# distributed-lab/linea-stark-prover

Hardware: AMD Instinct MI355X
Metric: prove time (s) + trace-rows/sec, 3x3 perm AIR @2^19; NTT HBM GB/s vs roofline (higher is better)
Workload: dtype fr253 (BLS12-377 Fr, 8x u32 Montgomery limbs); 1 GPU; 3x3 permutation AIR, 2^19 rows (w=8, q=4 quotient chunks, log_blowup 3, 33 queries, Poseidon2-w3 Merkle, FRI); log_n=19, width=8, fri_queries=33, parallelism=single-gpu

## Files before the change

linea_stark_prover_amd/csrc/capi.cpp:

```cpp
#include <hip/hip_runtime.h>

#include <algorithm>
#include <cstdlib>
#include <cstring>
#include <memory>
#include <thread>

#include "comm.hpp"
#include "prove_internal.hpp"

using namespace lsp;

namespace {
thread_local std::string g_err;

#ifdef LSP_DEBUG_BOUNDS
std::string bounds_fault_report() {
    int n = 0;
    if (hipGetDeviceCount(&n) != hipSuccess || n == 0) return "";
    (void)hipDeviceSynchronize();
    static const char* const files[] = {"k_ntt.hip", "k_hash.hip", "k_field.hip", "k_quotient.hip", "k_open.hip",
                                        "k_witness.hip", "k_check.hip", "fr29.hpp", "k_common.hpp", "poseidon2_f29.hpp",
                                        "fr.hpp"};
    static unsigned (*const readers[])() = {bounds_fault_k_ntt, bounds_fault_k_hash, bounds_fault_k_field,
// ... 92 lines not shown
                uint64_t x = next();
                c.v[2 * k] = (uint32_t)x;
                c.v[2 * k + 1] = (uint32_t)(x >> 32);
            }
            c.v[7] &= (1u << 29) - 1;
            if (fr_words_lt_mod(c)) return fr_from_canonical(c);
        }
    }
    uint64_t below(uint64_t n) {
        const unsigned __int128 two64 = (unsigned __int128)1 << 64;
        const unsigned __int128 lim = two64 - (two64 % n);
        for (;;) {
            uint64_t x = next();
            if ((unsigned __int128)x < lim) return x % n;
        }
    }
};
}

extern "C" {

#ifdef LSP_DEBUG_BOUNDS
const char* lsp_version(void) { return "linea_stark_prover_amd 0.1 (gfx950, debug-bounds)"; }
#else
const char* lsp_version(void) { return "linea_stark_prover_amd 0.1 (gfx950)"; }
#endif

int lsp_debug_bounds_probe(lsp_ctx* ctx) {
    return guarded(ctx, [&] {
        LSP_REQUIRE(ctx, LSP_E_ARG, "null ctx");
        std::lock_guard<std::mutex> g(ctx->mu);
        need_gpu(ctx);
#ifndef LSP_DEBUG_BOUNDS
        throw LspError(LSP_E_STATE, "not a debug-bounds build (python -m linea_stark_prover_amd.build --debug-bounds)");
#else
        uint32_t* sink = (uint32_t*)ctx->buf("bounds_probe", 4 * sizeof(uint32_t));
        LSP_HIP(launch_bounds_probe(sink, ctx->stream));
        ctx->sync();
#endif
    });
}

int lsp_device_count(int* n) {
    return guarded(nullptr, [&] {
        LSP_REQUIRE(n, LSP_E_ARG, "null");
        int c = 0;
        if (hipGetDeviceCount(&c) != hipSuccess) c = 0;
        *n = c;
    });
}

const char* lsp_last_error(const lsp_ctx* ctx) { return ctx ? ctx->err.c_str() : g_err.c_str(); }

int lsp_seeded_setup(uint64_t seed, uint32_t rounds_f, uint32_t rounds_p, lsp_fr* alpha, lsp_fr* delta,
                     lsp_fr* rc) {
    return guarded(nullptr, [&] {
        LSP_REQUIRE(alpha && delta && rc && rounds_f % 2 == 0, LSP_E_ARG, "bad seeded_setup arguments");
        SplitMix64 g{seed};
        *alpha = from_fr(g.fr());
        *delta = from_fr(g.fr());
        for (uint32_t i = 0; i < 3 * rounds_f + rounds_p; ++i) rc[i] = from_fr(g.fr());
    });
}

void lsp_fr_from_canonical(const uint64_t in[4], lsp_fr* out) {
    if (!in || !out) return;
    lsp_fr t;
    std::memcpy(t.l, in, 32);
    *out = from_fr(fr_from_canonical(to_fr(t)));
}
void lsp_fr_to_canonical(const lsp_fr* in, uint64_t out[4]) {
    if (!in || !out) return;
    lsp_fr t = from_fr(fr_to_canonical(to_fr(*in)));
    std::memcpy(out, t.l, 32);
}
void lsp_fr_from_be_bytes_mod_order(const uint8_t* be, size_t n, lsp_fr* out) {
    if (!out || (!be && n)) return;
    const Fr b256 = fr_from_u64(256);
    Fr acc = fr_zero();
    for (size_t i = 0; i < n; ++i) acc = fr_add(fr_mul(acc, b256), fr_from_u64(be[i]));
    *out = from_fr(acc);
}
void lsp_fr_mul(const lsp_fr* a, const lsp_fr* b, lsp_fr* out) {
    if (a && b && out) *out = from_fr(fr_mul(to_fr(*a), to_fr(*b))); }
void lsp_fr_inv(const lsp_fr* a, lsp_fr* out) {
    if (a && out) *out = from_fr(fr_inv(to_fr(*a)));
}
void lsp_two_adic_generator(uint32_t bits, lsp_fr* out) {
    if (!out) return;
    if (bits > 47) bits = 47;
    *out = from_fr(host_two_adic_generator(bits));
}

int lsp_ctx_create(int device, const lsp_params* p, lsp_ctx** out) {
    return guarded(nullptr, [&] {
        LSP_REQUIRE(p && out && p->round_constants, LSP_E_ARG, "null params");
        LSP_REQUIRE(p->struct_size == sizeof(lsp_params), LSP_E_ARG,
                    "lsp_params.struct_size must be sizeof(lsp_params) of this header (caller built against "
                    "another lsp.h?)");
        LSP_REQUIRE(p->skip_log_degree <= 1 && p->skip_public_values <= 1 && p->observe_opened_values <= 1 &&
                        p->sample_bits_montgomery <= 1 && p->skip_final_poly <= 1,
                    LSP_E_ARG, "transcript switches are 0 or 1");
        LSP_REQUIRE(p->sbox_degree == 11 || p->sbox_degree == 17, LSP_E_ARG, "S-box degree must be 11 or 17");
        LSP_REQUIRE(p->rounds_f >= 2 && p->rounds_f % 2 == 0 && p->rounds_f <= 64 && p->rounds_p <= 256, LSP_E_ARG,
                    "bad round counts");
        LSP_REQUIRE(p->log_blowup >= 1 && p->log_blowup <= 8 && p->num_queries >= 1 && p->num_queries <= 1024 &&
                        p->proof_of_work_bits <= 32 && p->log_final_poly_len <= 8 &&
                        (p->public_degree == 0 || p->public_degree == 1),
                    LSP_E_ARG, "bad FRI parameters");
        auto c = std::make_unique<lsp_ctx>();
        c->device = device;
        c->p2.L = P2Layout{p->rounds_f, p->rounds_p, p->sbox_degree};
        const size_t nround = 3 * p->rounds_f + p->rounds_p;
        const size_t nrc = nround + P2_LIN_N;
        c->p2.rc.resize(nrc);
        for (size_t i = 0; i < nround; ++i) c->p2.rc[i] = to_fr(p->round_constants[i]);
        {
            static const uint32_t dm[9] = {2, 1, 1, 1, 2, 1, 1, 1, 2}, dd[3] = {1, 1, 2};
            bool gen = false;
            for (int k = 0; k < 9; ++k) {
                const Fr def = fr_from_u64(dm[k]);
                Fr v = def;
                if (p->external_mds) {
                    v = to_fr(p->external_mds[k]);
                    LSP_REQUIRE(fr_words_lt_mod(v), LSP_E_ARG, "external_mds entry not canonical");
                }
                gen |= !fr_eq(v, def);
                c->p2.rc[nround + k] = v;
            }
            for (int k = 0; k < 3; ++k) {
                const Fr def = fr_from_u64(dd[k]);
                Fr v = def;
                if (p->internal_diag) {
                    v = to_fr(p->internal_diag[k]);
                    LSP_REQUIRE(fr_words_lt_mod(v), LSP_E_ARG, "internal_diag entry not canonical");
                }
                gen |= !fr_eq(v, def);
                c->p2.rc[nround + 9 + k] = v;
            }
            c->p2.L.gen_lin = gen ? 1u : 0u;
        }
        if (ifma::available()) ifma::prepare(c->p2.rc, c->p2.rc8);
        if (device != LSP_HOST_ONLY) {
            int n = 0;
            if (hipGetDeviceCount(&n) != hipSuccess || n == 0) throw LspError(LSP_E_STATE, "no HIP device");
            LSP_REQUIRE(device >= 0 && device < n, LSP_E_ARG, "bad device index");
            LSP_HIP(hipSetDevice(device));
            LSP_HIP(hipStreamCreateWithFlags(&c->stream, hipStreamNonBlocking));
            int lds = 0;
            if (hipDeviceGetAttribute(&lds, hipDeviceAttributeMaxSharedMemoryPerBlock, device) == hipSuccess && lds > 0)
                c->lds_per_block = (size_t)lds;
            LSP_HIP(hipMalloc(&c->rc_dev, nrc * sizeof(Fr)));
            LSP_HIP(hipMemcpy(c->rc_dev, c->p2.rc.data(), nrc * sizeof(Fr), hipMemcpyHostToDevice));
            LSP_HIP(hipMalloc(&c->rc29_dev, nrc * sizeof(F29)));
            LSP_HIP(launch_rc_to_f29(c->rc_dev, c->rc29_dev, (uint32_t)nrc, c->stream));
            LSP_HIP(hipStreamSynchronize(c->stream));
        }
        c->log_blowup = p->log_blowup;
        c->log_final_poly_len = p->log_final_poly_len;
        c->num_queries = p->num_queries;
        c->pow_bits = p->proof_of_work_bits;
        c->public_degree = p->public_degree;
        c->transcript.log_degree = !p->skip_log_degree;
        c->transcript.public_values = !p->skip_public_values;
        c->transcript.opened_values = p->observe_opened_values != 0;
        c->transcript.mont_bits = p->sample_bits_montgomery != 0;
        c->transcript.final_poly = !p->skip_final_poly;
        *out = c.release();
    });
}

int lsp_ctx_destroy(lsp_ctx* ctx) {
    if (!ctx) return LSP_OK;
    delete ctx->comm;
    ctx->comm = nullptr;
    if (ctx->device == LSP_HOST_ONLY) {
        delete ctx;
        return LSP_OK;
    }
    (void)hipSetDevice(ctx->device);
    (void)hipStreamSynchronize(ctx->stream);
    if (ctx->side_stream) (void)hipStreamSynchronize(ctx->side_stream);
    for (auto& kv : ctx->pool)
        if (kv.second.p) (void)hipFree(kv.second.p);
    for (auto& kv : ctx->hpool)
        if (kv.second.p) (void)hipHostFree(kv.second.p);
    for (auto& kv : ctx->twiddles) (void)hipFree(kv.second);
    for (auto& kv : ctx->stage_ev) (void)hipEventDestroy(kv.second);
    for (hipEvent_t e : ctx->event_pool) (void)hipEventDestroy(e);
    for (auto& t : ctx->pending_timings) {
        (void)hipEventDestroy(std::get<1>(t));
        (void)hipEventDestroy(std::get<2>(t));
    }
    if (ctx->ev_near) (void)hipEventDestroy(ctx->ev_near);
    if (ctx->ev_top) (void)hipEventDestroy(ctx->ev_top);
    if (ctx->ev_warm) (void)hipEventDestroy(ctx->ev_warm);
    if (ctx->side_stream) {
        (void)hipStreamSynchronize(ctx->side_stream);
        (void)hipEventDestroy(ctx->ev_wide);
        (void)hipEventDestroy(ctx->ev_side);
        (void)hipStreamDestroy(ctx->side_stream);
    }
    if (ctx->rc_dev) (void)hipFree(ctx->rc_dev);
    if (ctx->rc29_dev) (void)hipFree(ctx->rc29_dev);
    (void)hipStreamDestroy(ctx->stream);
    delete ctx;
    return LSP_OK;
}

int lsp_synchronize(lsp_ctx* ctx) {
    return guarded(ctx, [&] {
        LSP_REQUIRE(ctx, LSP_E_ARG, "null ctx");
        need_gpu(ctx);
        LSP_HIP(hipDeviceSynchronize());
    });
}

int lsp_dev_alloc(lsp_ctx* ctx, size_t bytes, void** dptr) {
    return guarded(ctx, [&] {
        LSP_REQUIRE(ctx && dptr, LSP_E_ARG, "null");
        need_gpu(ctx);
        if (hipMalloc(dptr, bytes ? bytes : 1) != hipSuccess) {
            (void)hipGetLastError();
            throw LspError(LSP_E_OOM, "hipMalloc failed");
        }
    });
}
int lsp_dev_free(lsp_ctx* ctx, void* dptr) {
    return guarded(ctx, [&] {
        need_gpu(ctx);
        LSP_HIP(hipFree(dptr));
    });
}
int lsp_memcpy_h2d(lsp_ctx* ctx, void* dst, const void* src, size_t bytes) {
    return guarded(ctx, [&] {
        LSP_REQUIRE(ctx && ((dst && src) || bytes == 0), LSP_E_ARG, "null memcpy argument");
        std::lock_guard<std::mutex> g(ctx->mu);
        need_gpu(ctx);
        LSP_HIP(hipMemcpyAsync(dst, src, bytes, hipMemcpyHostToDevice, ctx->stream));
        ctx->sync();
    });
}
int lsp_memcpy_d2h(lsp_ctx* ctx, void* dst, const void* src, size_t bytes) {
    return guarded(ctx, [&] {
        LSP_REQUIRE(ctx && ((dst && src) || bytes == 0), LSP_E_ARG, "null memcpy argument");
        std::lock_guard<std::mutex> g(ctx->mu);
        need_gpu(ctx);
        LSP_HIP(hipMemcpyAsync(dst, src, bytes, hipMemcpyDeviceToHost, ctx->stream));
        ctx->sync();
    });
}

int lsp_coset_lde_batch_shifts(lsp_ctx* ctx, const lsp_fr* in, size_t h, size_t w, uint32_t added_bits,
                               const lsp_fr* shifts, lsp_fr* out, int mem) {
    return guarded(ctx, [&] {
        LSP_REQUIRE(ctx && shifts && w >= 1, LSP_E_ARG, "bad arguments");
        std::lock_guard<std::mutex> g(ctx->mu);
        need_gpu(ctx);
        log2_exact(h);
        LSP_REQUIRE(added_bits <= 16, LSP_E_ARG, "added_bits too large");
        const size_t N = h << added_bits;
        std::vector<Fr> sh(w);
        for (size_t c = 0; c < w; ++c) sh[c] = to_fr(shifts[c]);
        const Fr* din = dev_in(ctx, in, h * w, mem, "api_in");
        Fr* dout = dev_out(ctx, out, N * w, mem, "api_out");
        lde_device(ctx, din, h, w, added_bits, sh.data(), dout);
        finish_out(ctx, out, dout, N * w, mem);
    });
}

int lsp_coset_lde_batch(lsp_ctx* ctx, const lsp_fr* in, size_t h, size_t w, uint32_t added_bits,
                        const lsp_fr* shift, lsp_fr* out, int mem) {
    if (!shift || w == 0) return LSP_E_ARG;
    std::vector<lsp_fr> sh(w, *shift);
    return lsp_coset_lde_batch_shifts(ctx, in, h, w, added_bits, sh.data(), out, mem);
}

int lsp_coset_dft_batch(lsp_ctx* ctx, const lsp_fr* coeffs, size_t h, size_t w, const lsp_fr* shift, lsp_fr* out,
                        int mem) {
    return guarded(ctx, [&] {
        LSP_REQUIRE(ctx && w >= 1, LSP_E_ARG, "bad dft arguments");
        std::lock_guard<std::mutex> g(ctx->mu);
        need_gpu(ctx);
        log2_exact(h);
        const Fr s = shift ? to_fr(*shift) : fr_one();
        const Fr* din = dev_in(ctx, coeffs, h * w, mem, "api_in");
        Fr* dout = dev_out(ctx, out, h * w, mem, "api_out");
        coset_dft_device(ctx, din, h, w, s, dout);
        finish_out(ctx, out, dout, h * w, mem);
    });
}

int lsp_coset_idft_batch(lsp_ctx* ctx, const lsp_fr* evals, size_t h, size_t w, const lsp_fr* shift, lsp_fr* out,
                         int mem) {
    return guarded(ctx, [&] {
        LSP_REQUIRE(ctx && w >= 1, LSP_E_ARG, "bad idft arguments");
        std::lock_guard<std::mutex> g(ctx->mu);
        need_gpu(ctx);
        log2_exact(h);
        const Fr s = shift ? to_fr(*shift) : fr_one();
        LSP_REQUIRE(!fr_is_zero(fr_to_canonical(s)), LSP_E_ARG, "coset shift must be nonzero");
        const Fr* din = dev_in(ctx, evals, h * w, mem, "api_in");
        Fr* dout = dev_out(ctx, out, h * w, mem, "api_out");
        coset_idft_device(ctx, din, h, w, s, dout);
        finish_out(ctx, out, dout, h * w, mem);
    });
}
// ... 1139 lines not shown
```

linea_stark_prover_amd/csrc/k_hash.hip:

```cpp
#include <cstdlib>

#include "k_common.hpp"
#include "kernels.hpp"
#include "poseidon2_f29.hpp"
#include "poseidon2_row.hpp"

namespace lsp {

#ifndef LSP_P2_ROWS_WPE
#define LSP_P2_ROWS_WPE 1
#endif

namespace {
template <uint32_t D>
__global__ __launch_bounds__(256) void k_permute(Fr* __restrict__ st, size_t n, const F29* __restrict__ rc,
                                                 uint32_t rf, uint32_t rp) {
    __shared__ uint4 qt[3 * F29_QTAB_N];
    f29_qtab_init(qt);
    __syncthreads();
    const size_t i = gtid();
    if (i >= n) return;
    F29 s0 = f29_from_fr(st[3 * i]), s1 = f29_from_fr(st[3 * i + 1]), s2 = f29_from_fr(st[3 * i + 2]);
    permute3_any<D, 1>(s0, s1, s2, rc, rf, rp, qt);
    st[3 * i] = f29_to_fr(s0);
    st[3 * i + 1] = f29_to_fr(s1);
    st[3 * i + 2] = f29_to_fr(s2);
}

template <uint32_t D, int LANES>
__global__ __launch_bounds__(256) __attribute__((amdgpu_waves_per_eu(LSP_P2_ROWS_WPE))) void k_hash_rows1(const Fr* __restrict__ m, uint32_t w, size_t nrows,
                                                    Fr* __restrict__ out, const F29* __restrict__ rc, uint32_t rf,
                                                    uint32_t rp) {
    __shared__ uint4 qt[3 * F29_QTAB_N];
    f29_qtab_init(qt);
    __syncthreads();
    const size_t i = gtid() / LANES;
    if (i >= nrows) return;
    const Fr* row = m + i * w;
    const Fr d = sponge_f29<D, LANES>([&](uint32_t k) { return LSP_BOUNDS(k < w) ? row[k] : fr_zero(); }, w, rc, rf,
                                      rp, qt);
    if ((threadIdx.x & (LANES - 1)) == 0) out[i] = d;
}

template <uint32_t D, int LANES>
__global__ __launch_bounds__(256) __attribute__((amdgpu_waves_per_eu(LSP_P2_ROWS_WPE))) void k_hash_rows_multi(MatList ml, size_t nrows, Fr* __restrict__ out,
                                                         const F29* __restrict__ rc, uint32_t rf, uint32_t rp) {
    __shared__ uint4 qt[3 * F29_QTAB_N];
    f29_qtab_init(qt);
    __syncthreads();
    const size_t i = gtid() / LANES;
    if (i >= nrows) return;
    uint32_t total = 0;
    for (uint32_t j = 0; j < ml.n; ++j) total += ml.width[j];
    auto get = [&](uint32_t k) {
        uint32_t j = 0;
        while (k >= ml.width[j]) {
            k -= ml.width[j];
            ++j;
            if (!LSP_BOUNDS(j < ml.n)) return fr_zero();
        }
        return ml.ptr[j][i * ml.width[j] + k];
    };
    const Fr d = sponge_f29<D, LANES>(get, total, rc, rf, rp, qt);
    if ((threadIdx.x & (LANES - 1)) == 0) out[i] = d;
}

template <uint32_t D, int LANES>
__global__ __launch_bounds__(256) void k_fold_hash(FoldSpec f, size_t nleaves, Fr* __restrict__ out,
                                                   const F29* __restrict__ rc, uint32_t rf, uint32_t rp) {
    __shared__ uint4 qt[3 * F29_QTAB_N];
    f29_qtab_init(qt);
    __syncthreads();
    const size_t j = gtid() / LANES;
    if (j >= nleaves) return;
    Fr e[2];
#pragma unroll
    for (int k = 0; k < 2; ++k) {
        const size_t i = 2 * j + k;
        const Fr p = fr_mul(f.half_beta, pow2l(f.tab, f.L1, brev_bits(f.i0 + i, f.logm)));
        e[k] = fr_add(fr_mul(fr_add(f.half, p), f.v[2 * i]), fr_mul(fr_sub(f.half, p), f.v[2 * i + 1]));
    }
    if ((threadIdx.x & (LANES - 1)) == 0) {
        f.vout[2 * j] = e[0];
        f.vout[2 * j + 1] = e[1];
    }
    const Fr d = sponge_f29<D, LANES>([&](uint32_t k) { return e[k]; }, 2, rc, rf, rp, qt);
    if ((threadIdx.x & (LANES - 1)) == 0) out[j] = d;
}

template <uint32_t D, int LANES>
__global__ __launch_bounds__(256) void k_merkle_level(const Fr* __restrict__ src, Fr* __restrict__ dst, size_t nout,
                                                      const F29* __restrict__ rc, uint32_t rf, uint32_t rp) {
    if constexpr (LANES > 1) __builtin_amdgcn_s_setprio(3);
    __shared__ uint4 qt[3 * F29_QTAB_N];
    f29_qtab_init(qt);
    __syncthreads();
    const size_t i = gtid() / LANES;
    if (i >= nout) return;
    if (!LSP_BOUNDS(2 * i + 1 < 2 * nout)) return;
    const Fr d = compress_f29<D, LANES>(src[2 * i], src[2 * i + 1], rc, rf, rp, qt);
    if ((threadIdx.x & (LANES - 1)) == 0) dst[i] = d;
}

template <uint32_t D>
__global__ __launch_bounds__(64) void k_merkle_level_row(const Fr* __restrict__ src, Fr* __restrict__ dst,
                                                         size_t nout, const F29* __restrict__ rc, uint32_t rf,
                                                         uint32_t rp) {
    __builtin_amdgcn_s_setprio(3);
    __shared__ prow::RowLds tab;
    prow::row_lds_init(&tab);
    __syncthreads();
    const size_t i = blockIdx.x;
    if (i >= nout) return;
    const Fr d = prow::compress_row<D>(src + 2 * i, src + 2 * i + 1, rc, rf, rp, &tab);
    if (threadIdx.x == 0) dst[i] = d;
}

template <uint32_t D>
__global__ __launch_bounds__(256) void k_merkle_top(Fr* __restrict__ layers, size_t off, uint32_t len,
                                                    const F29* __restrict__ rc, uint32_t rf, uint32_t rp) {
    __shared__ uint4 qt[3 * F29_QTAB_N];
    f29_qtab_init(qt);
    __syncthreads();
    __shared__ Fr buf[128];
    if (!LSP_BOUNDS(len <= 128)) return;
    for (uint32_t e = threadIdx.x; e < len; e += blockDim.x) buf[e] = layers[off + e];
    __syncthreads();
    size_t out_off = off + len;
    const uint32_t q = threadIdx.x >> 2;
    const bool lead = (threadIdx.x & 3) == 0;
    while (len > 1) {
        const uint32_t nout = len / 2;
        Fr r;
        if (q < nout) r = compress_f29<D, 4>(buf[2 * q], buf[2 * q + 1], rc, rf, rp, qt);
        __syncthreads();
        if (q < nout && lead) {
            buf[q] = r;
            layers[out_off + q] = r;
        }
        __syncthreads();
        out_off += nout;
        len = nout;
    }
}
template <uint32_t D>
__global__ __launch_bounds__(256) void k_grind(Fr pre0, Fr pre1, Fr pre2, uint32_t wlane, uint64_t base,
                                               uint64_t count, uint32_t bits, uint32_t mont, const F29* __restrict__ rc,
                                               uint32_t rf, uint32_t rp, unsigned long long* __restrict__ best) {
    __shared__ uint4 qt[3 * F29_QTAB_N];
    f29_qtab_init(qt);
    __syncthreads();
    const uint64_t stride = (uint64_t)gridDim.x * blockDim.x;
    const F29 c0 = f29_from_fr(pre0), c1 = f29_from_fr(pre1), c2 = f29_from_fr(pre2);
    const uint64_t mask = bits >= 64 ? ~0ull : ((1ull << bits) - 1);
    for (uint64_t i = gtid(); i < count; i += stride) {
        const uint64_t w = base + i;
        const F29 fw = f29_from_fr(fr_from_u64(w));
        F29 s0 = wlane == 0 ? fw : c0, s1 = wlane == 0 ? c1 : fw, s2 = c2;
        permute3_any<D, 1>(s0, s1, s2, rc, rf, rp, qt);
        const Fr m = f29_to_fr(s0);
        const Fr c = mont ? m : fr_to_canonical(m);
        const uint64_t lo = (uint64_t)c.v[0] | ((uint64_t)c.v[1] << 32);
        if ((lo & mask) == 0) atomicMin(best, (unsigned long long)w);
    }
}

template <uint32_t D>
__global__ __launch_bounds__(256) void k_calib_perm(Fr* __restrict__ out, uint32_t iters, const F29* __restrict__ rc,
                                                    uint32_t rf, uint32_t rp) {
    __shared__ uint4 qt[3 * F29_QTAB_N];
    f29_qtab_init(qt);
    __syncthreads();
    const size_t t = gtid();
    F29 s0 = f29_from_fr(fr_from_u64(t + 1)), s1 = f29_from_fr(fr_from_u64(3 * t + 7)), s2 = f29_zero();
    for (uint32_t i = 0; i < iters; ++i) permute3_any<D, 1>(s0, s1, s2, rc, rf, rp, qt);
    out[t] = f29_to_fr(s0);
}

__global__ void k_rc_to_f29(const Fr* __restrict__ rc, F29* __restrict__ rc29, uint32_t n) {
    const uint32_t i = (uint32_t)gtid();
    if (i < n) rc29[i] = f29_from_fr(rc[i]);
}
}

hipError_t launch_rc_to_f29(const Fr* rc, F29* rc29, uint32_t n, hipStream_t st) {
    hipLaunchKernelGGL(k_rc_to_f29, dim3(nblocks(n, 64)), dim3(64), 0, st, rc, rc29, n);
    return hipGetLastError();
}

#define LSP_DISPATCH_D(L, KERNEL, ...)                                  \
    do {                                                                \
        if ((L).gen_lin) {                                              \
            if ((L).sbox_degree == 17)                                  \
                hipLaunchKernelGGL(KERNEL<17u | P2_GEN>, __VA_ARGS__);  \
            else                                                        \
                hipLaunchKernelGGL(KERNEL<11u | P2_GEN>, __VA_ARGS__);  \
        } else if ((L).sbox_degree == 17)                               \
            hipLaunchKernelGGL(KERNEL<17>, __VA_ARGS__);                \
        else                                                            \
            hipLaunchKernelGGL(KERNEL<11>, __VA_ARGS__);                \
    } while (0)

#define LSP_DISPATCH_DL(DEG, LANES, KERNEL, ...)                          \
    do {                                                                  \
        if ((LANES) == 4)                                                 \
            hipLaunchKernelGGL((KERNEL<DEG, 4>), __VA_ARGS__);            \
        else if ((LANES) == 2)                                            \
            hipLaunchKernelGGL((KERNEL<DEG, 2>), __VA_ARGS__);            \
        else                                                              \
            hipLaunchKernelGGL((KERNEL<DEG, 1>), __VA_ARGS__);            \
    } while (0)
#define LSP_DISPATCH_DC(L, LANES, KERNEL, ...)                            \
    do {                                                                  \
        if ((L).gen_lin) {                                                \
            if ((L).sbox_degree == 17)                                    \
                LSP_DISPATCH_DL(17u | P2_GEN, LANES, KERNEL, __VA_ARGS__);\
            else                                                          \
                LSP_DISPATCH_DL(11u | P2_GEN, LANES, KERNEL, __VA_ARGS__);\
        } else if ((L).sbox_degree == 17)                                 \
            LSP_DISPATCH_DL(17u, LANES, KERNEL, __VA_ARGS__);             \
        else                                                              \
            LSP_DISPATCH_DL(11u, LANES, KERNEL, __VA_ARGS__);             \
    } while (0)

static size_t coop_max() {
    static const size_t v = [] {
        const char* e = std::getenv("LSP_COOP_MAX");
        return e ? (size_t)std::strtoull(e, nullptr, 10) : (size_t)16384;
    }();
    return v;
}
static unsigned coop_bs() {
    static const unsigned v = [] {
        const char* e = std::getenv("LSP_COOP_BS");
        return e ? (unsigned)std::strtoul(e, nullptr, 10) : 0u;
    }();
    return v;
}
#define COOP_MAX coop_max()
static size_t pair_max() {
    static const size_t v = [] {
        const char* e = std::getenv("LSP_PAIR_MAX");
        return e ? (size_t)std::strtoull(e, nullptr, 10) : (size_t)32768;
    }();
    return v;
}
static inline int lanes_for(size_t n) { return n <= COOP_MAX ? 4 : (n <= pair_max() ? 2 : 1); }

static inline void state_grid(size_t n, int lanes, unsigned& blocks, unsigned& bs) {
    if (lanes == 4) {
        bs = coop_bs() ? coop_bs() : (4 * n >= 65536 ? 256u : 64u);
        blocks = nblocks(4 * n, bs);
    } else {
        bs = 256;
        blocks = nblocks((size_t)lanes * n, bs);
    }
}

hipError_t launch_permute(Fr* states, size_t n, const F29* rc, P2Layout L, hipStream_t st) {
    if (!n) return hipSuccess;
    LSP_DISPATCH_D(L, k_permute, dim3(nblocks(n, 256)), dim3(256), 0, st, states, n, rc, L.rounds_f, L.rounds_p);
    return hipGetLastError();
}

hipError_t launch_hash_rows(const MatList& m, size_t nrows, Fr* out, const F29* rc, P2Layout L, hipStream_t st) {
    if (!nrows) return hipSuccess;
    const int lanes = lanes_for(nrows);
    unsigned blocks, bs;
    state_grid(nrows, lanes, blocks, bs);
    if (m.n == 1)
        LSP_DISPATCH_DC(L, lanes, k_hash_rows1, dim3(blocks), dim3(bs), 0, st, m.ptr[0], m.width[0], nrows, out, rc,
                        L.rounds_f, L.rounds_p);
    else
        LSP_DISPATCH_DC(L, lanes, k_hash_rows_multi, dim3(blocks), dim3(bs), 0, st, m, nrows, out, rc, L.rounds_f,
                        L.rounds_p);
    return hipGetLastError();
}

hipError_t launch_fold_hash(const FoldSpec& f, size_t nleaves, Fr* out, const F29* rc, P2Layout L, hipStream_t st) {
    if (!nleaves) return hipSuccess;
    const int lanes = lanes_for(nleaves);
    unsigned blocks, bs;
    state_grid(nleaves, lanes, blocks, bs);
    LSP_DISPATCH_DC(L, lanes, k_fold_hash, dim3(blocks), dim3(bs), 0, st, f, nleaves, out, rc, L.rounds_f, L.rounds_p);
    return hipGetLastError();
}

hipError_t launch_calib_perm(Fr* out, size_t nthreads, uint32_t iters, const F29* rc, P2Layout L, hipStream_t st) {
    LSP_DISPATCH_D(L, k_calib_perm, dim3(nblocks(nthreads, 256)), dim3(256), 0, st, out, iters, rc, L.rounds_f,
                   L.rounds_p);
    return hipGetLastError();
}

hipError_t launch_grind(const Fr pre[3], uint32_t wlane, uint64_t base, uint64_t count, uint32_t bits, bool mont,
                        const F29* rc, P2Layout L, unsigned long long* best, hipStream_t st) {
    const unsigned blocks = 256 * 16;
    LSP_DISPATCH_D(L, k_grind, dim3(blocks), dim3(256), 0, st, pre[0], pre[1], pre[2], wlane, base, count, bits,
                   (uint32_t)mont, rc,
                   L.rounds_f, L.rounds_p, best);
    return hipGetLastError();
}

static size_t row_max() {
    static const size_t v = [] {
        const char* e = std::getenv("LSP_ROW_MAX");
        return e ? (size_t)std::strtoull(e, nullptr, 10) : (size_t)1024;
    }();
    return v;
}

hipError_t launch_merkle_level(const Fr* src, Fr* dst, size_t nout, const F29* rc, P2Layout L, hipStream_t st) {
    if (!nout) return hipSuccess;
    if (!L.gen_lin && nout <= row_max()) {
        if (L.sbox_degree == 17)
            hipLaunchKernelGGL(k_merkle_level_row<17>, dim3((unsigned)nout), dim3(64), 0, st, src, dst, nout, rc,
                               L.rounds_f, L.rounds_p);
        else
            hipLaunchKernelGGL(k_merkle_level_row<11>, dim3((unsigned)nout), dim3(64), 0, st, src, dst, nout, rc,
                               L.rounds_f, L.rounds_p);
        return hipGetLastError();
    }
    const int lanes = lanes_for(nout);
    unsigned blocks, bs;
    state_grid(nout, lanes, blocks, bs);
    LSP_DISPATCH_DC(L, lanes, k_merkle_level, dim3(blocks), dim3(bs), 0, st, src, dst, nout, rc, L.rounds_f,
                    L.rounds_p);
    return hipGetLastError();
}

hipError_t launch_merkle_levels(Fr* layers, size_t nleaves, size_t stop_len, const F29* rc, P2Layout L,
                                size_t* off_out, size_t* len_out, hipStream_t st) {
    size_t off = 0, len = nleaves;
    while (len > stop_len && len > 1) {
        hipError_t e = launch_merkle_level(layers + off, layers + off + len, len / 2, rc, L, st);
        if (e != hipSuccess) return e;
        off += len;
        len /= 2;
    }
    *off_out = off;
    *len_out = len;
    return hipSuccess;
}

hipError_t launch_merkle_tree(Fr* layers, size_t nleaves, const F29* rc, P2Layout L, hipStream_t st) {
    size_t off = 0, len = nleaves;
    while (len > 128) {
        const size_t nout = len / 2;
        hipError_t e = launch_merkle_level(layers + off, layers + off + len, nout, rc, L, st);
        if (e != hipSuccess) return e;
        off += len;
        len /= 2;
    }
    if (len > 1) {
        LSP_DISPATCH_D(L, k_merkle_top, dim3(1), dim3(256), 0, st, layers, off, (uint32_t)len, rc, L.rounds_f,
                       L.rounds_p);
        return hipGetLastError();
    }
    return hipSuccess;
}

}

LSP_BOUNDS_READER(k_hash)
```

linea_stark_prover_amd/csrc/kernels.hpp:

```cpp
#pragma once
#include <hip/hip_runtime.h>
#include <stddef.h>
#include <stdint.h>

#include "fr.hpp"
#include "fr29.hpp"
#include "poseidon2.hpp"

namespace lsp {

constexpr uint32_t COLMAP_PLAIN = 0xffu;
struct ColMap {
    uint32_t logb = COLMAP_PLAIN;
    uint32_t stride = 0, c0 = 0, cstep = 1, valid = 0xffffffffu;
    uint32_t bw = 0;
    static ColMap plain(uint32_t w) {
        ColMap m;
        m.stride = w;
        m.valid = w;
        return m;
    }
    static ColMap blocked(uint32_t logb, uint32_t bw) {
        ColMap m;
        m.logb = logb;
        m.bw = bw;
        return m;
    }
};
hipError_t launch_lde(const Fr* in, Fr* X, Fr* out, size_t w, uint32_t logh, uint32_t ncosets, const uint4* tw_inv,
                      const uint4* tw_fwd, const Fr* twist, uint32_t L1, uint32_t L2, int twist_per_col,
                      const Fr* ratio, hipStream_t st);
hipError_t launch_intt(const Fr* in, ColMap map, Fr* X, size_t w, uint32_t logh, const uint4* tw_inv, hipStream_t st);
hipError_t launch_lde_coeffs(const Fr* coef, ColMap map, Fr* out, size_t w, uint32_t logh, uint32_t ncosets,
                             const uint4* tw_fwd, const Fr* twist, uint32_t L1, uint32_t L2, int twist_per_col,
                             const Fr* ratio, hipStream_t st);
hipError_t launch_fold_subcoset(const Fr* coef, ColMap map, size_t h, size_t S, uint32_t w, const Fr* fac, Fr* out,
                                hipStream_t st);
hipError_t launch_to_f29form(const Fr* in, Fr* out, size_t n, hipStream_t st);
hipError_t launch_scale_coeffs(const Fr* X, size_t h, uint32_t w, const Fr* tab, uint32_t L1, Fr* out,
                               hipStream_t st);
hipError_t launch_to_f29limbs(const Fr* in, uint4* out, size_t n, hipStream_t st);
hipError_t launch_stage_twiddles(const Fr* pw, uint32_t logH, uint4* out, hipStream_t st);
hipError_t launch_pow_tables(const Fr* bases, size_t nbases, uint32_t L1, uint32_t L2, const Fr* scale,
                             Fr* tabs, hipStream_t st);
hipError_t launch_powers(const Fr* tab, uint32_t L1, size_t n, Fr* out, hipStream_t st);

struct MatList {
    const Fr* ptr[8];
    uint32_t width[8];
    uint32_t n;
};
inline MatList one_mat(const Fr* p, uint32_t w) {
    MatList m{};
    m.ptr[0] = p;
    m.width[0] = w;
    m.n = 1;
    return m;
}
hipError_t launch_rc_to_f29(const Fr* rc, F29* rc29, uint32_t n, hipStream_t st);
hipError_t launch_permute(Fr* states, size_t n, const F29* rc29, P2Layout L, hipStream_t st);
struct FoldSpec {
    const Fr* v;
    Fr* vout;
    Fr half, half_beta;
    const Fr* tab;
    uint32_t L1, logm;
    uint64_t i0;
};
hipError_t launch_fold_hash(const FoldSpec& f, size_t nleaves, Fr* out, const F29* rc, P2Layout L, hipStream_t st);
hipError_t launch_hash_rows(const MatList& m, size_t nrows, Fr* out, const F29* rc29, P2Layout L, hipStream_t st);
hipError_t launch_merkle_level(const Fr* src, Fr* dst, size_t nout, const F29* rc29, P2Layout L, hipStream_t st);
hipError_t launch_grind(const Fr pre[3], uint32_t wlane, uint64_t base, uint64_t count, uint32_t bits, bool mont,
                        const F29* rc29, P2Layout L, unsigned long long* best, hipStream_t st);
hipError_t launch_merkle_tree(Fr* layers, size_t nleaves, const F29* rc29, P2Layout L, hipStream_t st);
hipError_t launch_merkle_levels(Fr* layers, size_t nleaves, size_t stop_len, const F29* rc29, P2Layout L,
                                size_t* off_out, size_t* len_out, hipStream_t st);

size_t batch_inverse_scratch(size_t n);
hipError_t launch_batch_inverse(const Fr* in, Fr* out, size_t n, hipStream_t st, Fr* scratch = nullptr,
                                const Fr* inv_total = nullptr);
hipError_t launch_calib_mul(Fr* out, size_t nthreads, uint32_t iters, hipStream_t st);
hipError_t launch_calib_perm(Fr* out, size_t nthreads, uint32_t iters, const F29* rc, P2Layout L, hipStream_t st);
hipError_t launch_gather(const uint64_t* ptrs, Fr* out, size_t n, hipStream_t st);
hipError_t launch_assemble_chunks(const Fr* stage, uint32_t logGq, size_t Sq, Fr* out, hipStream_t st);

size_t witness_scratch_bytes(size_t n, uint32_t ntables);
hipError_t launch_gen_raw_perm(uint64_t seed, size_t n, uint32_t ncols, uint64_t mul, uint64_t add, Fr* a, Fr* b,
                               hipStream_t st);
hipError_t launch_perm_rows(const Fr* a, uint32_t na, const Fr* b, uint32_t nb, size_t n, Fr alpha, Fr delta,
                            Fr* out, size_t ostride, Fr* al, Fr* bl, hipStream_t st);
hipError_t launch_lookup_rows(const Fr* a, uint32_t na, const Fr* b, uint32_t nt, uint32_t nbc, const Fr* afil,
                              const Fr* bfil, size_t n, Fr alpha, Fr delta, Fr* out, size_t ostride, Fr* comb,
                              Fr* den, hipStream_t st);
hipError_t launch_mul_vec(const Fr* x, const Fr* y, size_t n, Fr* out, hipStream_t st);
hipError_t launch_put_col(const Fr* v, size_t n, Fr* out, size_t ostride, uint32_t col, hipStream_t st);
hipError_t launch_fr_scan(const Fr* in, Fr* out, size_t n, bool product, void* scratch, size_t scratch_bytes,
                          hipStream_t st);
hipError_t launch_lookup_occurrences(const Fr* comb, size_t n, uint32_t nt, const Fr* afil, const Fr* bfil,
                                     uint32_t* occ, void* scratch, size_t scratch_bytes, hipStream_t st);
hipError_t launch_lookup_terms(const Fr* inv, const uint32_t* occ, const Fr* afil, size_t n, uint32_t nt, Fr* out,
                               size_t ostride, uint32_t col_ainv, Fr* term, hipStream_t st);

struct QuotientArgs {
    const Fr* lde;
    uint32_t w;
    uint32_t logQ, log_q;
    const int32_t* air;
    uint32_t air_len;
    Fr pub_alpha, pub_delta, alpha;
    Fr gen;
    Fr wh_inv;
    const Fr* tabQ;
    uint32_t L1;
    const Fr* zh;
    const Fr* inv_zh;
    const Fr* inv_den;
    Fr* out;
    uint64_t i0 = 0;
    uint32_t log_step = 0;
    uint64_t row0 = 0;
    uint64_t n = 0;
    const Fr* lde_next = nullptr;
    uint64_t row0_next = 0;
    uint32_t row_order = 0;
    uint64_t lde_rows = 0, lde_next_rows = 0;
    uint32_t* cons = nullptr;
    uint32_t ncons = 0;
    const Fr* pub = nullptr;
    uint32_t npub = 0;
    uint32_t prog = 0, prog_slots = 0;
    const Fr* prep = nullptr;
    uint32_t wp = 0;
};
hipError_t launch_selector_denoms(const Fr* tabQ, uint32_t L1, Fr gen, Fr wh_inv, size_t n, Fr* den,
                                  hipStream_t st, uint64_t i0 = 0, uint32_t log_step = 0);
hipError_t launch_quotient(const QuotientArgs& a, hipStream_t st);
hipError_t launch_quotient_fold(const QuotientArgs& a, hipStream_t st);

struct CheckArgs {
    const Fr* trace;
    uint64_t h;
    uint32_t w;
    const int32_t* air;
    uint32_t ncons;
    Fr pub_alpha, pub_delta;
    uint64_t* row_mask;
    uint64_t* count;
    uint64_t* first_row;
    const uint64_t* rows = nullptr;
    uint32_t nrows = 0;
    Fr* vals = nullptr;
    const Fr* pub = nullptr;
    uint32_t npub = 0;
    uint32_t prog = 0, prog_slots = 0;
    const Fr* prep = nullptr;
    uint32_t wp = 0;
};
hipError_t launch_check(const CheckArgs& a, hipStream_t st);
hipError_t launch_check_rows(const CheckArgs& a, hipStream_t st);

hipError_t launch_open_denoms(Fr z, Fr gen, const Fr* tabN, uint32_t L1, uint32_t logN, size_t n, Fr* den,
                              hipStream_t st, uint64_t row0 = 0);
hipError_t launch_shift_inverse(const Fr* inv_z, Fr* out, Fr c, uint32_t logN, uint64_t step, uint64_t row0, size_t n,
                                hipStream_t st);
hipError_t launch_interp_partial(const Fr* M, uint32_t w, size_t h, const Fr* inv_den, Fr gen, const Fr* tabN,
                                 uint32_t L1, uint32_t logN, Fr* partial, uint32_t* nblocks, hipStream_t st,
                                 uint64_t row0 = 0);
hipError_t launch_sum_partials(const Fr* partial, uint32_t nblocks, uint32_t w, Fr* out, hipStream_t st);
struct ReduceArgs {
    const Fr* lde;
    uint32_t w;
    const Fr* qlde;
    uint32_t q;
    const Fr* inv_z;
    const Fr* inv_zn;
    const Fr* apw;
    Fr ry_z, ry_zn;
    const Fr* ryq;
    Fr* out;
    size_t n;
    F29* consts29 = nullptr;
    size_t lds_max = 64 * 1024;
};
inline size_t reduce_rows_scratch(uint32_t w, uint32_t q, size_t lds_max) {
    const size_t lds = 3 * 64 * 16 + (w + 1 + 2 * (size_t)q) * 36;
    return lds <= lds_max ? 0 : w + 1 + 2 * (size_t)q;
}
hipError_t launch_reduce_rows(const ReduceArgs& a, hipStream_t st);
struct PrepReduceArgs {
    const Fr* prep;
    uint32_t wp;
    const Fr* inv_z;
    const Fr* inv_zn;
    const Fr* apw;
    Fr ry_z, ry_zn, off_z, off_zn;
    Fr* out;
    size_t n;
    size_t lds_max = 64 * 1024;
};
bool reduce_prep_fits(uint32_t wp, size_t lds_max);
hipError_t launch_reduce_prep(const PrepReduceArgs& a, hipStream_t st);
hipError_t launch_bounds_probe(uint32_t* sink, hipStream_t st);
#ifdef LSP_DEBUG_BOUNDS
unsigned bounds_fault_k_ntt();
unsigned bounds_fault_k_hash();
unsigned bounds_fault_k_field();
unsigned bounds_fault_k_quotient();
unsigned bounds_fault_k_open();
unsigned bounds_fault_k_witness();
unsigned bounds_fault_k_check();
#endif
// ... 7 lines not shown
```

linea_stark_prover_amd/csrc/poseidon2_row.hpp:

```cpp
#pragma once
#include "poseidon2_f29.hpp"

namespace lsp {
#include "fr29_row_gfx950.inc"

namespace prow {

__device__ __forceinline__ uint32_t shr1(uint32_t x) {
    return (uint32_t)__builtin_amdgcn_mov_dpp((int)x, 0x111, 0xf, 0xf, true);
}
__device__ __forceinline__ uint32_t bcast8(uint32_t x) {
    return (uint32_t)__builtin_amdgcn_mov_dpp((int)x, 0x158, 0xf, 0xf, false);
}
__device__ __forceinline__ void swap16(uint32_t& a, uint32_t& b) {
    const auto r = __builtin_amdgcn_permlane16_swap(a, b, false, false);
    a = r[0];
    b = r[1];
}
__device__ __forceinline__ void swap32(uint32_t& a, uint32_t& b) {
    const auto r = __builtin_amdgcn_permlane32_swap(a, b, false, false);
    a = r[0];
    b = r[1];
}
__device__ __forceinline__ uint32_t rowsum(uint32_t x) {
    uint32_t a = x, b = x;
    swap16(a, b);
    uint32_t s = a + b, t = s;
    swap32(s, t);
    return s + t;
}
__device__ __forceinline__ uint32_t row0_all(uint32_t x) {
    uint32_t a = x, b = x;
    swap16(a, b);
    uint32_t c = a;
    swap32(a, c);
    return a;
}
__device__ __forceinline__ uint32_t row1_all(uint32_t x) {
    uint32_t a = x, b = x;
    swap16(a, b);
    uint32_t c = b;
    swap32(b, c);
    return b;
}
__device__ __forceinline__ uint32_t row2_all(uint32_t x) {
    uint32_t a = x, b = x;
    swap32(a, b);
    uint32_t c = b;
    swap16(b, c);
    return b;
}

struct Lane {
    F29RowK K;
    uint32_t l;
    uint32_t row;
    bool hi9;
};

__device__ __forceinline__ uint32_t rnorm(uint32_t v, const Lane& L) {
#pragma unroll
    for (int k = 0; k < 2; ++k) v = (v & L.K.maskl) + shr1(v >> 29);
    return L.hi9 ? 0u : v;
}

struct RowLds {
    uint32_t rqt[16 * F29_QTAB_N];
    uint32_t ptab[32];
    uint32_t c0[16];
    uint32_t cto[16];
};

__device__ __forceinline__ void row_lds_init(RowLds* t) {
    for (uint32_t q = threadIdx.x; q < F29_QTAB_N; q += blockDim.x) {
        uint32_t Q[9];
        uint64_t c = 0;
#pragma unroll
        for (int i = 0; i < 8; ++i) {
            const uint64_t v = (uint64_t)q * p29(i) + c;
            Q[i] = (uint32_t)v & F29_MASK;
            c = v >> 29;
        }
        Q[8] = (uint32_t)((uint64_t)q * p29(8) + c);
        uint32_t* e = t->rqt + 16 * q;
        const uint32_t b = q ? 2u : 0u;
        e[0] = q ? (1u << 30) - Q[0] : 0u;
#pragma unroll
        for (int i = 1; i < 8; ++i) e[i] = q ? (1u << 30) - b - Q[i] : 0u;
        e[8] = 0u - b - Q[8];
#pragma unroll
        for (int i = 9; i < 16; ++i) e[i] = 0u;
    }
    constexpr uint32_t TO[9] = {0x1ffffff3u, 0x8e3ffffu, 0x1ffffc9fu, 0xfea1edfu, 0xfee725u,
                                0xabaa896u,  0xa745b60u, 0x6457773u,  0xd4bdau};
    for (uint32_t i = threadIdx.x; i < 32; i += blockDim.x) {
        uint32_t v = 0;
#pragma unroll
        for (int d = 1; d <= 8; ++d) v = i == 8u + d ? p29(d) : v;
        t->ptab[i] = v;
        if (i < 16) {
            uint32_t c = 0, o = 0;
#pragma unroll
            for (int l = 0; l < 9; ++l) {
                c = i == (uint32_t)l ? c29(l) : c;
                o = i == (uint32_t)l ? TO[l] : o;
            }
            t->c0[i] = c;
            t->cto[i] = o;
        }
    }
}

__device__ __forceinline__ Lane row_lane(const RowLds* t) {
    Lane L;
    const uint32_t lane = threadIdx.x & 63u;
    L.l = lane & 15u;
    L.row = lane >> 4;
    L.hi9 = L.l >= 9;
    L.K.c0 = t->c0[L.l];
#pragma unroll
    for (int k = 0; k < 9; ++k) L.K.P[k] = t->ptab[8 + L.l - k];
    L.K.maskl = L.l == 8 ? 0xffffffffu : F29_MASK;
    return L;
}

__device__ __forceinline__ uint32_t rq_entry(uint32_t v, const uint32_t* __restrict__ rqt, const Lane& L) {
    uint32_t q = __umulhi(bcast8(v), 0xdb651d12u) >> 20;
    if (!LSP_BOUNDS(q < F29_QTAB_N)) q = 0;
    q = q ? q - 1 : 0u;
    return rqt[16 * q + L.l];
}
__device__ __forceinline__ uint32_t rreduce(uint32_t v, const uint32_t* __restrict__ rqt, const Lane& L) {
    return rnorm(v + rq_entry(v, rqt, L), L);
}

__device__ __forceinline__ uint32_t rmul(uint32_t a, uint32_t b, const Lane& L) { return f29row_mul(a, b, L.K); }

template <uint32_t D>
__device__ __forceinline__ uint32_t sbox(uint32_t x, const Lane& L) {
    const uint32_t x2 = rmul(x, x, L);
    const uint32_t x4 = rmul(x2, x2, L);
    const uint32_t x8 = rmul(x4, x4, L);
    if (D == 11) return rmul(rmul(x8, x2, L), x, L);
    return rmul(rmul(x8, x8, L), x, L);
}

__device__ __forceinline__ uint32_t load_limb(const Fr* p, const Lane& L) {
    if (L.hi9) return 0u;
    const uint32_t* w = reinterpret_cast<const uint32_t*>(p);
    const uint32_t b = 29 * L.l + 27, W = b >> 5;
    const uint32_t lo = W ? w[W - 1] : 0u, hi = W < 8 ? w[W] : 0u;
    const uint32_t v = __builtin_amdgcn_alignbit(hi, lo, b & 31);
    return L.l < 8 ? v & F29_MASK : v;
}

__device__ __forceinline__ uint32_t rc_limb(const F29* __restrict__ rc29, uint32_t k, const Lane& L) {
    return L.hi9 ? 0u : rc29[k].l[L.l];
}

template <uint32_t D>
__device__ __forceinline__ Fr compress_row(const Fr* left, const Fr* right, const F29* __restrict__ rc29, uint32_t rf,
                                           uint32_t rp, const RowLds* __restrict__ tab) {
    const Lane L = row_lane(tab);
    const uint32_t* rqt = tab->rqt;
    const uint32_t half = rf / 2;
    const F29* ini = rc29;
    const F29* ter = rc29 + 3 * half;
    const F29* itl = rc29 + 6 * half;
    uint32_t S = L.row == 0 ? load_limb(left, L) : L.row == 1 ? load_limb(right, L) : 0u;
    S = rreduce(S, rqt, L);
    uint32_t T = rowsum(S);
    const bool live = L.row < 3;
    uint32_t C = live ? rc_limb(ini, L.row, L) : 0u;
    for (uint32_t r = 0; r < half; ++r) {
        const uint32_t x = rnorm(S + C + T, L);
        C = live && r + 1 < half ? rc_limb(ini, 3 * (r + 1) + L.row, L) : 0u;
        const uint32_t y = sbox<D>(x, L);
        S = live ? y : 0u;
        T = rowsum(S);
    }
    const uint32_t W = S + T;
    uint32_t Ci = rp ? rc_limb(itl, 0, L) : 0u;
    uint32_t X = row0_all(rnorm(W + Ci, L));
    const uint32_t R = rreduce(W, rqt, L);
    uint32_t S1 = row1_all(R), S2 = row2_all(R);
    const bool odd = L.row & 1u;
    uint32_t v1 = S1, v2 = S2, e1 = 0, e2 = 0;
    for (uint32_t r = 0; r < rp; ++r) {
        Ci = r + 1 < rp ? rc_limb(itl, r + 1, L) : 0u;
        const uint32_t x2 = rmul(X, X, L);
        S1 = rnorm(v1 + e1, L);
        S2 = rnorm(v2 + e2, L);
        uint32_t y;
        if (D == 11) {
            uint32_t a = rmul(x2, odd ? X : x2, L);
            uint32_t b = a;
            swap16(a, b);
            y = rmul(rmul(a, a, L), b, L);
        } else {
            const uint32_t x4 = rmul(x2, x2, L);
            const uint32_t x8 = rmul(x4, x4, L);
            y = rmul(rmul(x8, x8, L), X, L);
        }
        const uint32_t u = y + S1 + S2;
        v1 = S1 + u;
        v2 = S2 + S2 + u;
        e1 = rq_entry(v1, rqt, L);
        e2 = rq_entry(v2, rqt, L);
        X = rnorm(y + Ci + u, L);
    }
    S1 = rnorm(v1 + e1, L);
    S2 = rnorm(v2 + e2, L);
    S = L.row == 0 ? X : L.row == 1 ? S1 : L.row == 2 ? S2 : 0u;
    T = 0;
    C = live ? rc_limb(ter, L.row, L) : 0u;
    for (uint32_t r = 0; r < half; ++r) {
        const uint32_t x = rnorm(S + C + T, L);
        C = live && r + 1 < half ? rc_limb(ter, 3 * (r + 1) + L.row, L) : 0u;
        const uint32_t y = sbox<D>(x, L);
        S = live ? y : 0u;
        T = rowsum(S);
    }
    const uint32_t y = rmul(rnorm(S + T, L), tab->cto[L.l], L);
    F29 o;
#pragma unroll
    for (int i = 0; i < 9; ++i) o.l[i] = __builtin_amdgcn_readlane(y, i);
    return fr_reduce_once(f29_repack_out(f29_reduce(o)));
}

}
}
```

Measured before the change: 8.675 million trace-rows/s.

## Precompute row-hash LDS table once and prefetch fold/merkle inputs before table init

```diff
diff --git a/linea_stark_prover_amd/csrc/capi.cpp b/linea_stark_prover_amd/csrc/capi.cpp
--- a/linea_stark_prover_amd/csrc/capi.cpp
+++ b/linea_stark_prover_amd/csrc/capi.cpp
@@ -268,7 +268,7 @@
                 c->lds_per_block = (size_t)lds;
             LSP_HIP(hipMalloc(&c->rc_dev, nrc * sizeof(Fr)));
             LSP_HIP(hipMemcpy(c->rc_dev, c->p2.rc.data(), nrc * sizeof(Fr), hipMemcpyHostToDevice));
-            LSP_HIP(hipMalloc(&c->rc29_dev, nrc * sizeof(F29)));
+            LSP_HIP(hipMalloc(&c->rc29_dev, rc29_bytes(nrc)));
             LSP_HIP(launch_rc_to_f29(c->rc_dev, c->rc29_dev, (uint32_t)nrc, c->stream));
             LSP_HIP(hipStreamSynchronize(c->stream));
         }
diff --git a/linea_stark_prover_amd/csrc/k_hash.hip b/linea_stark_prover_amd/csrc/k_hash.hip
--- a/linea_stark_prover_amd/csrc/k_hash.hip
+++ b/linea_stark_prover_amd/csrc/k_hash.hip
@@ -69,16 +69,44 @@
 __global__ __launch_bounds__(256) void k_fold_hash(FoldSpec f, size_t nleaves, Fr* __restrict__ out,
                                                    const F29* __restrict__ rc, uint32_t rf, uint32_t rp) {
     __shared__ uint4 qt[3 * F29_QTAB_N];
-    f29_qtab_init(qt);
-    __syncthreads();
+    Fr e[2];
+    if constexpr (LANES > 1) {
+        const size_t j = gtid() / LANES;
+        const bool live = j < nleaves;
+        const size_t jl = live ? j : 0;
+        Fr v[4], tl[2], th[2];
+#pragma unroll
+        for (int k = 0; k < 2; ++k) {
+            const size_t i = 2 * jl + k;
+            const uint64_t x = brev_bits(f.i0 + i, f.logm);
+            uint64_t hi = x >> f.L1;
+            if (!LSP_BOUNDS(hi < (1ull << f.L1))) hi = 0;
+            tl[k] = f.tab[x & ((1ull << f.L1) - 1)];
+            th[k] = f.tab[(1ull << f.L1) + hi];
+            v[2 * k] = f.v[2 * i];
+            v[2 * k + 1] = f.v[2 * i + 1];
+        }
+        f29_qtab_init(qt);
+        __syncthreads();
+        if (!live) return;
+#pragma unroll
+        for (int k = 0; k < 2; ++k) {
+            const Fr p = fr_mul(f.half_beta, fr_mul(tl[k], th[k]));
+            e[k] = fr_add(fr_mul(fr_add(f.half, p), v[2 * k]), fr_mul(fr_sub(f.half, p), v[2 * k + 1]));
+        }
+    } else {
+        f29_qtab_init(qt);
+        __syncthreads();
+    }
     const size_t j = gtid() / LANES;
     if (j >= nleaves) return;
-    Fr e[2];
+    if constexpr (LANES == 1) {
 #pragma unroll
-    for (int k = 0; k < 2; ++k) {
-        const size_t i = 2 * j + k;
-        const Fr p = fr_mul(f.half_beta, pow2l(f.tab, f.L1, brev_bits(f.i0 + i, f.logm)));
-        e[k] = fr_add(fr_mul(fr_add(f.half, p), f.v[2 * i]), fr_mul(fr_sub(f.half, p), f.v[2 * i + 1]));
+        for (int k = 0; k < 2; ++k) {
+            const size_t i = 2 * j + k;
+            const Fr p = fr_mul(f.half_beta, pow2l(f.tab, f.L1, brev_bits(f.i0 + i, f.logm)));
+            e[k] = fr_add(fr_mul(fr_add(f.half, p), f.v[2 * i]), fr_mul(fr_sub(f.half, p), f.v[2 * i + 1]));
+        }
     }
     if ((threadIdx.x & (LANES - 1)) == 0) {
         f.vout[2 * j] = e[0];
@@ -105,16 +133,21 @@
 template <uint32_t D>
 __global__ __launch_bounds__(64) void k_merkle_level_row(const Fr* __restrict__ src, Fr* __restrict__ dst,
                                                          size_t nout, const F29* __restrict__ rc, uint32_t rf,
-                                                         uint32_t rp) {
+                                                         uint32_t rp, const prow::RowLds* __restrict__ gtab) {
     __builtin_amdgcn_s_setprio(3);
     __shared__ prow::RowLds tab;
-    prow::row_lds_init(&tab);
-    __syncthreads();
     const size_t i = blockIdx.x;
     if (i >= nout) return;
-    const Fr d = prow::compress_row<D>(src + 2 * i, src + 2 * i + 1, rc, rf, rp, &tab);
+    const prow::RowTabRegs t = prow::row_tab_fetch(gtab);
+    const uint32_t S = prow::load_state(src + 2 * i, src + 2 * i + 1);
+    prow::row_tab_store(&tab, t);
+    __syncthreads();
+    const Fr d = prow::compress_row_state<D>(S, rc, rf, rp, &tab);
     if (threadIdx.x == 0) dst[i] = d;
 }
+
+__global__ __launch_bounds__(64) void k_row_tab_init(prow::RowLds* __restrict__ g) { prow::row_lds_init(g); }
+static_assert(sizeof(prow::RowLds) == P2_ROW_TAB_BYTES, "kernels.hpp sizes the context's buffer for it");
 
 template <uint32_t D>
 __global__ __launch_bounds__(256) void k_merkle_top(Fr* __restrict__ layers, size_t off, uint32_t len,
@@ -185,6 +218,8 @@
 
 hipError_t launch_rc_to_f29(const Fr* rc, F29* rc29, uint32_t n, hipStream_t st) {
     hipLaunchKernelGGL(k_rc_to_f29, dim3(nblocks(n, 64)), dim3(64), 0, st, rc, rc29, n);
+    hipLaunchKernelGGL(k_row_tab_init, dim3(1), dim3(64), 0, st,
+                       reinterpret_cast<prow::RowLds*>(reinterpret_cast<char*>(rc29) + rc29_tab_offset(n)));
     return hipGetLastError();
 }
 
@@ -312,12 +347,14 @@
 hipError_t launch_merkle_level(const Fr* src, Fr* dst, size_t nout, const F29* rc, P2Layout L, hipStream_t st) {
     if (!nout) return hipSuccess;
     if (!L.gen_lin && nout <= row_max()) {
+        const auto* gtab = reinterpret_cast<const prow::RowLds*>(reinterpret_cast<const char*>(rc) +
+                                                                 rc29_tab_offset(p2_lin_offset(L) + P2_LIN_N));
         if (L.sbox_degree == 17)
             hipLaunchKernelGGL(k_merkle_level_row<17>, dim3((unsigned)nout), dim3(64), 0, st, src, dst, nout, rc,
-                               L.rounds_f, L.rounds_p);
+                               L.rounds_f, L.rounds_p, gtab);
         else
             hipLaunchKernelGGL(k_merkle_level_row<11>, dim3((unsigned)nout), dim3(64), 0, st, src, dst, nout, rc,
-                               L.rounds_f, L.rounds_p);
+                               L.rounds_f, L.rounds_p, gtab);
         return hipGetLastError();
     }
     const int lanes = lanes_for(nout);
diff --git a/linea_stark_prover_amd/csrc/kernels.hpp b/linea_stark_prover_amd/csrc/kernels.hpp
--- a/linea_stark_prover_amd/csrc/kernels.hpp
+++ b/linea_stark_prover_amd/csrc/kernels.hpp
@@ -57,6 +57,9 @@
     m.n = 1;
     return m;
 }
+constexpr size_t P2_ROW_TAB_BYTES = 4352;
+inline size_t rc29_tab_offset(size_t n) { return (n * sizeof(F29) + 15) & ~(size_t)15; }
+inline size_t rc29_bytes(size_t n) { return rc29_tab_offset(n) + P2_ROW_TAB_BYTES; }
 hipError_t launch_rc_to_f29(const Fr* rc, F29* rc29, uint32_t n, hipStream_t st);
 hipError_t launch_permute(Fr* states, size_t n, const F29* rc29, P2Layout L, hipStream_t st);
 struct FoldSpec {
diff --git a/linea_stark_prover_amd/csrc/poseidon2_row.hpp b/linea_stark_prover_amd/csrc/poseidon2_row.hpp
--- a/linea_stark_prover_amd/csrc/poseidon2_row.hpp
+++ b/linea_stark_prover_amd/csrc/poseidon2_row.hpp
@@ -64,12 +64,34 @@
     return L.hi9 ? 0u : v;
 }
 
-struct RowLds {
+struct alignas(16) RowLds {
     uint32_t rqt[16 * F29_QTAB_N];
     uint32_t ptab[32];
     uint32_t c0[16];
     uint32_t cto[16];
 };
+
+struct RowTabRegs {
+    uint4 q[4];
+    uint32_t w;
+};
+static_assert(sizeof(RowLds) == 4 * 64 * sizeof(uint4) + 64 * sizeof(uint32_t), "row_tab_fetch's split");
+
+__device__ __forceinline__ RowTabRegs row_tab_fetch(const RowLds* __restrict__ g) {
+    const uint4* gq = reinterpret_cast<const uint4*>(g->rqt);
+    RowTabRegs t;
+#pragma unroll
+    for (int k = 0; k < 4; ++k) t.q[k] = gq[64 * k + threadIdx.x];
+    t.w = reinterpret_cast<const uint32_t*>(g)[16 * F29_QTAB_N + threadIdx.x];
+    return t;
+}
+
+__device__ __forceinline__ void row_tab_store(RowLds* t, const RowTabRegs& r) {
+    uint4* q = reinterpret_cast<uint4*>(t->rqt);
+#pragma unroll
+    for (int k = 0; k < 4; ++k) q[64 * k + threadIdx.x] = r.q[k];
+    reinterpret_cast<uint32_t*>(t)[16 * F29_QTAB_N + threadIdx.x] = r.w;
+}
 
 __device__ __forceinline__ void row_lds_init(RowLds* t) {
     for (uint32_t q = threadIdx.x; q < F29_QTAB_N; q += blockDim.x) {
@@ -145,13 +167,14 @@
     return rmul(rmul(x8, x8, L), x, L);
 }
 
-__device__ __forceinline__ uint32_t load_limb(const Fr* p, const Lane& L) {
-    if (L.hi9) return 0u;
-    const uint32_t* w = reinterpret_cast<const uint32_t*>(p);
-    const uint32_t b = 29 * L.l + 27, W = b >> 5;
-    const uint32_t lo = W ? w[W - 1] : 0u, hi = W < 8 ? w[W] : 0u;
-    const uint32_t v = __builtin_amdgcn_alignbit(hi, lo, b & 31);
-    return L.l < 8 ? v & F29_MASK : v;
+__device__ __forceinline__ uint32_t load_state(const Fr* left, const Fr* right) {
+    const uint32_t lane = threadIdx.x & 63u, l = lane & 15u, row = lane >> 4;
+    const uint32_t* w = reinterpret_cast<const uint32_t*>(row == 1 ? right : left);
+    const uint32_t b = 29 * min(l, 8u) + 27, W = b >> 5;
+    const uint32_t wl = w[W ? W - 1 : 0], wh = w[min(W, 7u)];
+    const uint32_t v = __builtin_amdgcn_alignbit(W < 8 ? wh : 0u, W ? wl : 0u, b & 31);
+    const uint32_t m = (row < 2 && l < 9) ? (l < 8 ? F29_MASK : 0xffffffffu) : 0u;
+    return v & m;
 }
 
 __device__ __forceinline__ uint32_t rc_limb(const F29* __restrict__ rc29, uint32_t k, const Lane& L) {
@@ -159,15 +182,14 @@
 }
 
 template <uint32_t D>
-__device__ __forceinline__ Fr compress_row(const Fr* left, const Fr* right, const F29* __restrict__ rc29, uint32_t rf,
-                                           uint32_t rp, const RowLds* __restrict__ tab) {
+__device__ __forceinline__ Fr compress_row_state(uint32_t S, const F29* __restrict__ rc29, uint32_t rf, uint32_t rp,
+                                                 const RowLds* __restrict__ tab) {
     const Lane L = row_lane(tab);
     const uint32_t* rqt = tab->rqt;
     const uint32_t half = rf / 2;
     const F29* ini = rc29;
     const F29* ter = rc29 + 3 * half;
     const F29* itl = rc29 + 6 * half;
-    uint32_t S = L.row == 0 ? load_limb(left, L) : L.row == 1 ? load_limb(right, L) : 0u;
     S = rreduce(S, rqt, L);
     uint32_t T = rowsum(S);
     const bool live = L.row < 3;
@@ -228,5 +250,11 @@
     return fr_reduce_once(f29_repack_out(f29_reduce(o)));
 }
 
-}
-}
+template <uint32_t D>
+__device__ __forceinline__ Fr compress_row(const Fr* left, const Fr* right, const F29* __restrict__ rc29, uint32_t rf,
+                                           uint32_t rp, const RowLds* __restrict__ tab) {
+    return compress_row_state<D>(load_state(left, right), rc29, rf, rp, tab);
+}
+
+}
+}
```

Result: no change. 8.695 million trace-rows/s, median of 3 (+0.2%).
